# svip-lab/impersonator

Hardware: NVIDIA H100
Metric: frames/sec @256x256 (per-frame inference hot path) (higher is better)
Workload: dtype f16 main product + e4m3 correction products (hi/lo split), f32 accumulate

## Files before the change

impersonator_b200/csrc/conv_tc.cu:

```cuda
#include <cuda.h>

#include <stdlib.h>

#include <algorithm>
#include <new>

#include "common.cuh"

namespace {

constexpr int TILE_H = 16, TILE_W = 8;
constexpr int SWAP_N_TILE = 64;
constexpr int SWAP_TILE_H = 32;
constexpr int KCHUNK = 64;
constexpr int ROW_BYTES = TILE_W * 128;
constexpr int MAX_TAPS = 49;
constexpr int MAX_GROUP = 8;
constexpr int RING_BYTES = 200 * 1024;
constexpr int MAX_STAGES = 8;
constexpr int NUM_CONSUMERS = 256;
constexpr int NUM_THREADS = NUM_CONSUMERS + 32;
constexpr int MAX_N_TILE = 128;
static_assert(2 * 2 * (TILE_H + MAX_GROUP - 1) * ROW_BYTES + 2 * 2 * MAX_N_TILE * 128 <= RING_BYTES,
              "every plan needs two A and two B entries in the ring");
static_assert(2 * 2 * (SWAP_TILE_H + MAX_GROUP - 1) * ROW_BYTES + 2 * 2 * SWAP_N_TILE * 128 <= RING_BYTES,
              "every swapped plan needs two A and two B entries in the ring");
static_assert(SWAP_N_TILE * (SWAP_TILE_H * TILE_W) == MAX_N_TILE * (TILE_H * TILE_W), "same accumulator budget");

__host__ __device__ constexpr int tile_rows(int n_tile) { return n_tile == SWAP_N_TILE ? SWAP_TILE_H : TILE_H; }

struct ConvParams {
    CUtensorMap a_hi[4];
    CUtensorMap a_lo[4];
    CUtensorMap w_hi;
    CUtensorMap w_lo;
    int n_img, tiles_y, tiles_x, n_tiles_n;
    int dom_h, dom_w;
    int ntaps, chunks0, chunks1;
    signed char dy[MAX_TAPS], dx[MAX_TAPS], tmap[MAX_TAPS];
    short wtap[MAX_TAPS];
    int ngroups;
    signed char g_first[MAX_TAPS], g_cnt[MAX_TAPS];
    int a_rows;
    int a_stages, b_stages;
    float* out; int out_h, out_w, cout;
    int oy_mul, oy_add, ox_mul, ox_add;
    double* stats;
    float out_scale;
    int phase_cols;
};

template <int N_TILE, bool SPLIT>
struct Cfg {
    static constexpr int B_BYTES = N_TILE * 128;
    static constexpr int B_STAGE_BYTES = B_BYTES * (SPLIT ? 2 : 1);
    static constexpr int BAR_BYTES = 4 * MAX_STAGES * 8;
    static constexpr int STATS_BYTES = 8 * N_TILE * 8;
    static constexpr int SMEM_BYTES = 1024 + RING_BYTES + BAR_BYTES + STATS_BYTES;
    static_assert(B_STAGE_BYTES % 1024 == 0, "B entries must keep the 1024-byte swizzle alignment");
    static_assert(SMEM_BYTES <= 227 * 1024, "exceeds the shared memory of a block");
};

__device__ __forceinline__ uint32_t smem_u32(const void* p) { return (uint32_t)__cvta_generic_to_shared(p); }

__device__ __forceinline__ void mbar_init(uint64_t* bar, uint32_t count) {
    asm volatile("mbarrier.init.shared::cta.b64 [%0], %1;" ::"r"(smem_u32(bar)), "r"(count));
}
__device__ __forceinline__ void mbar_expect_tx(uint64_t* bar, uint32_t bytes) {
    asm volatile("mbarrier.arrive.expect_tx.shared::cta.b64 _, [%0], %1;" ::"r"(smem_u32(bar)), "r"(bytes) : "memory");
}
__device__ __forceinline__ void mbar_arrive(uint64_t* bar) {
    asm volatile("mbarrier.arrive.shared::cta.b64 _, [%0];" ::"r"(smem_u32(bar)) : "memory");
// ... 61 lines not shown
}
template <> __device__ __forceinline__ void wgmma_e4m3<16>(float* d, uint64_t da, uint64_t db) {
    asm volatile("{\n\t.reg .pred p;\n\tsetp.ne.b32 p, %10, 0;\n\t"
                 "wgmma.mma_async.sync.aligned.m64n16k32.f32.e4m3.e4m3 {%0, %1, %2, %3, %4, %5, %6, %7}, %8, %9, p, 1, 1;\n\t}"
                 : "+f"(d[0]), "+f"(d[1]), "+f"(d[2]), "+f"(d[3]), "+f"(d[4]), "+f"(d[5]), "+f"(d[6]), "+f"(d[7])
                 : "l"(da), "l"(db), "r"(1));
}
template <> __device__ __forceinline__ void wgmma_e4m3<32>(float* d, uint64_t da, uint64_t db) {
    asm volatile("{\n\t.reg .pred p;\n\tsetp.ne.b32 p, %18, 0;\n\t"
                 "wgmma.mma_async.sync.aligned.m64n32k32.f32.e4m3.e4m3 {%0, %1, %2, %3, %4, %5, %6, %7, %8, %9, %10, %11, %12, %13, %14, %15}, %16, %17, p, 1, 1;\n\t}"
                 : "+f"(d[0]), "+f"(d[1]), "+f"(d[2]), "+f"(d[3]), "+f"(d[4]), "+f"(d[5]), "+f"(d[6]), "+f"(d[7]), "+f"(d[8]), "+f"(d[9]), "+f"(d[10]), "+f"(d[11]), "+f"(d[12]), "+f"(d[13]), "+f"(d[14]), "+f"(d[15])
                 : "l"(da), "l"(db), "r"(1));
}
template <> __device__ __forceinline__ void wgmma_e4m3<128>(float* d, uint64_t da, uint64_t db) {
    asm volatile("{\n\t.reg .pred p;\n\tsetp.ne.b32 p, %66, 0;\n\t"
                 "wgmma.mma_async.sync.aligned.m64n128k32.f32.e4m3.e4m3 {%0, %1, %2, %3, %4, %5, %6, %7, %8, %9, %10, %11, %12, %13, %14, %15, %16, %17, %18, %19, %20, %21, %22, %23, %24, %25, %26, %27, %28, %29, %30, %31, %32, %33, %34, %35, %36, %37, %38, %39, %40, %41, %42, %43, %44, %45, %46, %47, %48, %49, %50, %51, %52, %53, %54, %55, %56, %57, %58, %59, %60, %61, %62, %63}, %64, %65, p, 1, 1;\n\t}"
                 : "+f"(d[0]), "+f"(d[1]), "+f"(d[2]), "+f"(d[3]), "+f"(d[4]), "+f"(d[5]), "+f"(d[6]), "+f"(d[7]), "+f"(d[8]), "+f"(d[9]), "+f"(d[10]), "+f"(d[11]), "+f"(d[12]), "+f"(d[13]), "+f"(d[14]), "+f"(d[15]), "+f"(d[16]), "+f"(d[17]), "+f"(d[18]), "+f"(d[19]), "+f"(d[20]), "+f"(d[21]), "+f"(d[22]), "+f"(d[23]), "+f"(d[24]), "+f"(d[25]), "+f"(d[26]), "+f"(d[27]), "+f"(d[28]), "+f"(d[29]), "+f"(d[30]), "+f"(d[31]), "+f"(d[32]), "+f"(d[33]), "+f"(d[34]), "+f"(d[35]), "+f"(d[36]), "+f"(d[37]), "+f"(d[38]), "+f"(d[39]), "+f"(d[40]), "+f"(d[41]), "+f"(d[42]), "+f"(d[43]), "+f"(d[44]), "+f"(d[45]), "+f"(d[46]), "+f"(d[47]), "+f"(d[48]), "+f"(d[49]), "+f"(d[50]), "+f"(d[51]), "+f"(d[52]), "+f"(d[53]), "+f"(d[54]), "+f"(d[55]), "+f"(d[56]), "+f"(d[57]), "+f"(d[58]), "+f"(d[59]), "+f"(d[60]), "+f"(d[61]), "+f"(d[62]), "+f"(d[63])
                 : "l"(da), "l"(db), "r"(1));
}

__device__ __forceinline__ void consumer_sync() { asm volatile("bar.sync 1, 256;" ::: "memory"); }

struct TileCoord {
    int n_idx, img, y0, x0;
};
template <int TH>
__device__ __forceinline__ TileCoord decode_tile(const ConvParams& P, int tile, int m_tiles) {
    TileCoord t;
    t.n_idx = tile / m_tiles;
    const int m_idx = tile % m_tiles;
    t.img = m_idx / (P.tiles_y * P.tiles_x);
    const int rem = m_idx % (P.tiles_y * P.tiles_x);
    t.y0 = (rem / P.tiles_x) * TH; t.x0 = (rem % P.tiles_x) * TILE_W;
    return t;
}

template <int N_TILE>
__device__ __forceinline__ void warp_tile_stats(const float* acc, bool v0, bool v1, int warp, unsigned lane, float2* s_stats)
{
#pragma unroll
    for (int j = 0; j < N_TILE / 8; j++) {
        const float a0 = v0 ? acc[4 * j] : 0.f, a1 = v0 ? acc[4 * j + 1] : 0.f;
        const float b0 = v1 ? acc[4 * j + 2] : 0.f, b1 = v1 ? acc[4 * j + 3] : 0.f;
        float s0 = a0 + b0, s1 = a1 + b1, q0 = a0 * a0 + b0 * b0, q1 = a1 * a1 + b1 * b1;
#pragma unroll
        for (int off = 4; off <= 16; off <<= 1) {
            s0 += __shfl_xor_sync(0xffffffffu, s0, off); s1 += __shfl_xor_sync(0xffffffffu, s1, off);
            q0 += __shfl_xor_sync(0xffffffffu, q0, off); q1 += __shfl_xor_sync(0xffffffffu, q1, off);
        }
        if (lane < 4) {
            s_stats[warp * N_TILE + 8 * j + 2 * lane] = make_float2(s0, q0);
            s_stats[warp * N_TILE + 8 * j + 2 * lane + 1] = make_float2(s1, q1);
        }
    }
}

template <int N_TILE, int PARTS = 8>
__device__ __forceinline__ void flush_tile_stats(const ConvParams& P, const float2* s_stats, int img, int n_idx)
{
    consumer_sync();
    for (int col = threadIdx.x; col < N_TILE; col += NUM_CONSUMERS) {
        float s = 0.f, q = 0.f;
#pragma unroll
        for (int w = 0; w < PARTS; w++) { const float2 v = s_stats[w * N_TILE + col]; s += v.x; q += v.y; }
        int ch = n_idx * N_TILE + col;
        if (P.phase_cols > 0) ch %= P.phase_cols;
        double* dst = P.stats + 2 * ((size_t)img * P.cout + ch);
        atomicAdd(dst, (double)s);
        atomicAdd(dst + 1, (double)q);
    }
    consumer_sync();
}

template <int N_TILE>
__device__ __forceinline__ void epilogue_plain(const ConvParams& P, float* acc, const TileCoord& t, int warp, unsigned lane,
                                               float2* s_stats)
{
    const int tx = (int)(lane >> 2), x = t.x0 + tx;
    const int y[2] = {t.y0 + 2 * warp, t.y0 + 2 * warp + 1};
    const bool valid[2] = {y[0] < P.dom_h && x < P.dom_w, y[1] < P.dom_h && x < P.dom_w};
    if (P.out_scale != 1.f) {
#pragma unroll
        for (int i = 0; i < N_TILE / 2; i++) acc[i] *= P.out_scale;
    }
    if (P.out) {
        const int out_w_c = P.out_w * P.cout;
#pragma unroll
        for (int h = 0; h < 2; h++) {
            if (!valid[h]) continue;
            float* optr = P.out + (((size_t)t.img * P.out_h + (P.oy_mul * y[h] + P.oy_add)) * P.out_w + (P.ox_mul * x + P.ox_add)) * P.cout
                        + (size_t)t.n_idx * N_TILE;
#pragma unroll
            for (int j = 0; j < N_TILE / 8; j++) {
                const int c = 8 * j + 2 * (int)(lane & 3);
                float* o = optr + c;
                if (P.phase_cols > 0) {
                    const int col = t.n_idx * N_TILE + c, ph = col / P.phase_cols;
                    o = P.out + (((size_t)t.img * P.out_h + 2 * y[h]) * P.out_w + 2 * x) * P.cout
                      + (size_t)(ph >> 1) * out_w_c + (ph & 1) * P.cout + (col - ph * P.phase_cols);
                }
                *reinterpret_cast<float2*>(o) = make_float2(acc[4 * j + 2 * h], acc[4 * j + 2 * h + 1]);
            }
        }
    }
    if (P.stats) {
        warp_tile_stats<N_TILE>(acc, valid[0], valid[1], warp, lane, s_stats);
        flush_tile_stats<N_TILE>(P, s_stats, t.img, t.n_idx);
    }
}

__device__ __forceinline__ void epilogue_swapped(const ConvParams& P, float* acc, const TileCoord& t, int warp, unsigned lane,
                                                 float2* s_stats)
{
    constexpr int N = SWAP_N_TILE;
    const int wg = warp >> 2;
    const int c0 = 16 * (warp & 3) + (int)(lane >> 2);
    const int y0 = t.y0 + 16 * wg, x0 = t.x0 + 2 * (int)(lane & 3);
    const int rows = P.dom_h - y0;
    const bool vx[2] = {x0 < P.dom_w, x0 + 1 < P.dom_w};
    if (P.out_scale != 1.f) {
#pragma unroll
        for (int i = 0; i < 64; i++) acc[i] *= P.out_scale;
    }
    if (P.out) {
        float* obase = P.out + (size_t)t.n_idx * N + c0;
#pragma unroll
        for (int j = 0; j < 16; j++) {
            if (j >= rows) break;
            const size_t orow = ((size_t)t.img * P.out_h + (P.oy_mul * (y0 + j) + P.oy_add)) * P.out_w;
#pragma unroll
            for (int e = 0; e < 2; e++) {
                if (!vx[e]) continue;
                float* o = obase + (orow + (P.ox_mul * (x0 + e) + P.ox_add)) * P.cout;
                o[0] = acc[4 * j + e];
                o[8] = acc[4 * j + 2 + e];
            }
        }
    }
    if (P.stats) {
        float s[2] = {0.f, 0.f}, q[2] = {0.f, 0.f};
#pragma unroll
        for (int j = 0; j < 16; j++) {
#pragma unroll
            for (int e = 0; e < 2; e++) {
                const bool v = j < rows && vx[e];
#pragma unroll
                for (int h = 0; h < 2; h++) {
                    const float a = v ? acc[4 * j + 2 * h + e] : 0.f;
                    s[h] += a; q[h] += a * a;
                }
            }
        }
#pragma unroll
        for (int h = 0; h < 2; h++) {
#pragma unroll
            for (int off = 1; off <= 2; off <<= 1) {
// ... 36 lines not shown
    const int a_stage_bytes = a_op_bytes * (SPLIT ? 2 : 1);
    uint8_t* b_ring = smem + P.a_stages * a_stage_bytes;
    uint64_t* a_full = reinterpret_cast<uint64_t*>(smem + RING_BYTES);
    uint64_t* a_empty = a_full + MAX_STAGES;
    uint64_t* b_full = a_empty + MAX_STAGES;
    uint64_t* b_empty = b_full + MAX_STAGES;
    float2* s_stats = reinterpret_cast<float2*>(smem + RING_BYTES + C::BAR_BYTES);

    const int warp = threadIdx.x >> 5;
    const unsigned lane = threadIdx.x & 31;

    if (threadIdx.x == 0) {
        for (int s = 0; s < P.a_stages; s++) { mbar_init(a_full + s, 1); mbar_init(a_empty + s, NUM_CONSUMERS / 32); }
        for (int s = 0; s < P.b_stages; s++) { mbar_init(b_full + s, 1); mbar_init(b_empty + s, NUM_CONSUMERS / 32); }
        fence_barrier_init();
        fence_proxy_async();
    }
    __syncthreads();
    lwb::pdl_wait();
    lwb::pdl_trigger();

    const int nchunks = P.chunks0 + P.chunks1;
    const int m_tiles = P.n_img * P.tiles_y * P.tiles_x;
    const int total = m_tiles * P.n_tiles_n;

    if (warp == NUM_CONSUMERS / 32) {
        if (elect_one()) {
            asm volatile("prefetch.tensormap [%0];" :: "l"(&P.a_hi[0]) : "memory");
            asm volatile("prefetch.tensormap [%0];" :: "l"(&P.w_hi) : "memory");
            if (SPLIT) {
                asm volatile("prefetch.tensormap [%0];" :: "l"(&P.a_lo[0]) : "memory");
                asm volatile("prefetch.tensormap [%0];" :: "l"(&P.w_lo) : "memory");
            }
        }
        int as = 0, bs = 0; uint32_t aph = 0, bph = 0;
        for (int tile = blockIdx.x; tile < total; tile += gridDim.x) {
            const TileCoord t = decode_tile<TH>(P, tile, m_tiles);
            for (int g = 0; g < P.ngroups; g++) {
                const int first = P.g_first[g], cnt = P.g_cnt[g];
                const int xx = t.x0 + P.dx[first], yy = t.y0 + P.dy[first];
                for (int chunk = 0; chunk < nchunks; chunk++) {
                    const bool second = chunk >= P.chunks0;
                    const int mi = second ? 1 : P.tmap[first];
                    const int c0 = (second ? chunk - P.chunks0 : chunk) * KCHUNK;
                    mbar_wait(a_empty + as, aph ^ 1);
                    uint8_t* sa = smem + as * a_stage_bytes;
                    if (elect_one()) {
                        mbar_expect_tx(a_full + as, (uint32_t)a_stage_bytes);
                        tma_load_4d(&P.a_hi[mi], sa, a_full + as, c0, xx, yy, t.img);
                        if (SPLIT) tma_load_4d(&P.a_lo[mi], sa + a_op_bytes, a_full + as, c0, xx, yy, t.img);
                    }
                    __syncwarp();
                    if (++as == P.a_stages) { as = 0; aph ^= 1; }
                    for (int i = 0; i < cnt; i++) {
                        mbar_wait(b_empty + bs, bph ^ 1);
                        uint8_t* sb = b_ring + bs * C::B_STAGE_BYTES;
                        const int wt = P.wtap[first + i];
                        if (elect_one()) {
                            mbar_expect_tx(b_full + bs, (uint32_t)C::B_STAGE_BYTES);
                            tma_load_3d(&P.w_hi, sb, b_full + bs, chunk * KCHUNK, t.n_idx * N_TILE, wt);
                            if (SPLIT) tma_load_3d(&P.w_lo, sb + C::B_BYTES, b_full + bs, chunk * KCHUNK, t.n_idx * N_TILE, wt);
                        }
                        __syncwarp();
                        if (++bs == P.b_stages) { bs = 0; bph ^= 1; }
                    }
                }
            }
        }
    } else if (warp < NUM_CONSUMERS / 32) {
        const uint32_t smem_base = smem_u32(smem);
        const uint32_t b_base = smem_u32(b_ring);
        const uint32_t a_row0 = (uint32_t)(warp >> 2) * (TH / 2) * ROW_BYTES;
        float acc[ACC];
        float acc8[MODE == MODE_F8 ? ACC : 1];
        int as = 0, bs = 0; uint32_t aph = 0, bph = 0;
        for (int tile = blockIdx.x; tile < total; tile += gridDim.x) {
            const TileCoord t = decode_tile<TH>(P, tile, m_tiles);
#pragma unroll
            for (int i = 0; i < ACC; i++) acc[i] = 0.f;
#pragma unroll
            for (int i = 0; i < (MODE == MODE_F8 ? ACC : 1); i++) acc8[i] = 0.f;
            int prev_b = -1, prev_a = -1;
            for (int g = 0; g < P.ngroups; g++) {
                const int cnt = P.g_cnt[g];
                for (int chunk = 0; chunk < nchunks; chunk++) {
                    mbar_wait(a_full + as, aph);
                    const uint32_t a_hi = smem_base + as * a_stage_bytes + a_row0;
                    for (int i = 0; i < cnt; i++) {
                        mbar_wait(b_full + bs, bph);
                        const uint32_t ai = a_hi + i * ROW_BYTES, al = ai + a_op_bytes;
                        const uint32_t b_hi = b_base + bs * C::B_STAGE_BYTES, b_lo = b_hi + C::B_BYTES;
                        wgmma_fence();
#pragma unroll
                        for (int k = 0; k < KCHUNK / 16; k++) {
                            const uint64_t da = make_desc(ai + k * 32), db = make_desc(b_hi + k * 32);
                            mma_f16<N_TILE, SWAP>(acc, da, db);
                            if constexpr (MODE == MODE_F8) {
                                mma_e4m3<N_TILE, SWAP>(acc8, make_desc(al + k * 32), make_desc(b_lo + k * 32));
                            } else if constexpr (MODE == MODE_FP16X3) {
                                mma_f16<N_TILE, SWAP>(acc, da, make_desc(b_lo + k * 32));
                                mma_f16<N_TILE, SWAP>(acc, make_desc(al + k * 32), db);
                            }
                        }
                        wgmma_commit();
                        if (prev_b >= 0) {
                            wgmma_wait<1>();
// ... 96 lines not shown
    switch (L.n_tile) {
        case 16:  return launch_one<16>(L, st);
        case 32:  return launch_one<32>(L, st);
        case 64:  return launch_one<64>(L, st);
        case 128: return launch_one<128>(L, st);
    }
    lwb::set_error("conv_tc: unsupported N tile %d", L.n_tile);
    return LWB_E_UNSUPPORTED;
}

int pick_n_tile(int cout, int forced)
{
    if (forced > 0) return forced > MAX_N_TILE && forced % MAX_N_TILE == 0 ? MAX_N_TILE : forced;
    if (cout % 128 == 0) return 128;
    if (cout % 64 == 0) return 64;
    if (cout % 32 == 0) return 32;
    if (cout % 16 == 0) return 16;
    return -1;
}

}

struct lwb_conv_plan {
    int num;
    Launch launches[4];
};

static int map_nhwc(CUtensorMap* m, const uint16_t* base, int n, int h, int w, int c, int rows)
{
    const uint64_t dims[4] = {(uint64_t)c, (uint64_t)w, (uint64_t)h, (uint64_t)n};
    const uint64_t str[3] = {(uint64_t)c * 2, (uint64_t)w * c * 2, (uint64_t)h * w * c * 2};
    const uint32_t box[4] = {(uint32_t)KCHUNK, TILE_W, (uint32_t)rows, 1};
    return encode_map(m, base, 4, dims, str, box);
}
static int map_nhwc_parity(CUtensorMap* m, const uint16_t* base, int n, int h, int w, int c, int py, int px, int rows)
{
    const uint64_t dims[4] = {(uint64_t)c, (uint64_t)((w - px + 1) / 2), (uint64_t)((h - py + 1) / 2), (uint64_t)n};
    const uint64_t str[3] = {(uint64_t)2 * c * 2, (uint64_t)2 * w * c * 2, (uint64_t)h * w * c * 2};
    const uint32_t box[4] = {(uint32_t)KCHUNK, TILE_W, (uint32_t)rows, 1};
    return encode_map(m, base + ((size_t)py * w + px) * c, 4, dims, str, box);
}

static void group_taps(ConvParams& p, int tile_h)
{
    int order[MAX_TAPS];
    for (int t = 0; t < p.ntaps; t++) order[t] = t;
    std::stable_sort(order, order + p.ntaps, [&](int a, int b) {
        if (p.tmap[a] != p.tmap[b]) return p.tmap[a] < p.tmap[b];
        if (p.dx[a] != p.dx[b]) return p.dx[a] < p.dx[b];
        return p.dy[a] < p.dy[b];
    });
    const ConvParams src = p;
    int longest = 0;
    p.ngroups = 0;
    for (int t = 0; t < p.ntaps; t++) {
        const int o = order[t];
        p.dy[t] = src.dy[o]; p.dx[t] = src.dx[o]; p.tmap[t] = src.tmap[o]; p.wtap[t] = src.wtap[o];
        const bool joins = t > 0 && p.tmap[t] == p.tmap[t - 1] && p.dx[t] == p.dx[t - 1] && p.dy[t] == p.dy[t - 1] + 1 &&
                           p.g_cnt[p.ngroups - 1] < MAX_GROUP;
        if (!joins) { p.g_first[p.ngroups] = (signed char)t; p.g_cnt[p.ngroups] = 0; p.ngroups++; }
        p.g_cnt[p.ngroups - 1]++;
        longest = std::max(longest, (int)p.g_cnt[p.ngroups - 1]);
    }
    p.a_rows = tile_h + longest - 1;
}

static void pick_rings(ConvParams& p, int n_tile, bool split)
{
    const int ops = split ? 2 : 1;
    const int a_bytes = p.a_rows * ROW_BYTES * ops, b_bytes = n_tile * 128 * ops;
    const int longest = p.a_rows - tile_rows(n_tile) + 1;
    int best = 0;
    for (int a = 2; a <= MAX_STAGES; a++) {
        const int b = std::min(MAX_STAGES, (RING_BYTES - a * a_bytes) / b_bytes);
        if (b < 2) break;
        if (std::min(a * longest, b) > best) { best = std::min(a * longest, b); p.a_stages = a; p.b_stages = b; }
    }
}

extern "C" int lwb_conv_plan_create(const lwb_conv_desc* d,
                                    const uint16_t* x0_hi, const uint16_t* x0_lo,
                                    const uint16_t* x1_hi, const uint16_t* x1_lo,
                                    const uint16_t* w_hi, const uint16_t* w_lo,
                                    float* out_raw, double* stats, lwb_conv_plan** plan_out)
{
    LWB_CHECK_ARG(d && x0_hi && w_hi && out_raw && plan_out, "null pointer");
    const bool split = d->split != 0;
    const bool f8 = d->split == 2;
    LWB_CHECK_ARG(d->split >= 0 && d->split <= 2, "split must be 0, 1 or 2");
    LWB_CHECK_ARG(!split || (x0_lo && w_lo), "split mode needs the lo operands");
    LWB_CHECK_ARG(!f8 || (!d->rowk && !d->halo), "the fp8 lo mode is not available for row-K / halo plans");
    LWB_CHECK_ARG(d->n > 0 && d->h_in > 0 && d->w_in > 0 && d->cout > 0, "non-positive size");
    LWB_CHECK_ARG(d->cout % 16 == 0, "cout must be a multiple of 16");
    LWB_CHECK_ARG(!f8 || (d->w_exp >= -40 && d->w_exp <= 60), "w_exp out of range");
    int n_tile = pick_n_tile(d->cout, d->n_tile);
    LWB_CHECK_ARG(n_tile > 0 && d->cout % n_tile == 0, "no N tile divides cout");
    if (d->halo) {
        LWB_CHECK_ARG(d->stride == 1 && !d->transposed && d->dil == 1, "halo mode needs stride 1, dilation 1, not transposed");
        if (d->rowk) LWB_CHECK_ARG(d->kw <= 8 && d->cin0 == 8 && d->cin1 == 0 && d->row_pitch >= d->w_in + 8, "row-K shape");
        else         LWB_CHECK_ARG(d->kw <= 9 && (d->kw & 1) && (d->kh & 1), "halo mode needs an odd kernel, kw <= 9, with 'same' padding (kh/2, kw/2)");
    }

    const int sms = lwb::sm_count();
    lwb_conv_plan* plan = new (std::nothrow) lwb_conv_plan();
    LWB_CHECK_ARG(plan, "out of host memory");
    plan->num = 0;
    int rc = LWB_OK;
    auto fail = [&](int code) { delete plan; return code; };

    auto finish = [&](Launch& L, int dom_h, int dom_w) {
        ConvParams& p = L.p;
        p.n_img = d->n;
        p.dom_h = dom_h; p.dom_w = dom_w;
        p.tiles_y = lwb::ceil_div(dom_h, tile_rows(n_tile)); p.tiles_x = lwb::ceil_div(dom_w, TILE_W);
        p.n_tiles_n = d->cout / n_tile;
        p.out = out_raw; p.out_h = d->h_out; p.out_w = d->w_out; p.cout = d->cout;
        p.stats = stats;
        p.out_scale = f8 ? ldexpf(1.f, -d->w_exp) : 1.f;
        L.n_tile = n_tile; L.mode = d->split;
        pick_rings(p, n_tile, split);
        const long total = (long)p.n_img * p.tiles_y * p.tiles_x * p.n_tiles_n;
        L.grid = (int)(total < sms ? total : sms);
    };

    if (d->rowk) {
        LWB_CHECK_ARG(d->stride == 1 && !d->transposed && d->kw <= 8 && d->cin0 == 8 && d->cin1 == 0, "row-K needs stride 1, kw <= 8, 8 channels");
        LWB_CHECK_ARG(d->h_out == d->h_in && d->w_out == d->w_in && d->row_pitch >= d->w_in + 8, "row-K shape");
        Launch& L = plan->launches[plan->num++];
        memset(&L.p, 0, sizeof(L.p));
        L.p.ntaps = d->kh; L.p.chunks0 = 1; L.p.chunks1 = 0;
        for (int ky = 0; ky < d->kh; ky++) { L.p.dy[ky] = (signed char)ky; L.p.dx[ky] = 0; L.p.tmap[ky] = 0; L.p.wtap[ky] = (short)ky; }
        group_taps(L.p, tile_rows(n_tile));
        const int hp = d->h_in + d->kh - 1;
        const uint64_t dims[4] = {64, (uint64_t)d->w_in, (uint64_t)hp, (uint64_t)d->n};
        const uint64_t str[3] = {16, (uint64_t)d->row_pitch * 16, (uint64_t)hp * d->row_pitch * 16};
        const uint32_t box[4] = {KCHUNK, TILE_W, (uint32_t)L.p.a_rows, 1};
        if ((rc = encode_map(&L.p.a_hi[0], x0_hi, 4, dims, str, box)) != LWB_OK) return fail(rc);
        if (split && (rc = encode_map(&L.p.a_lo[0], x0_lo, 4, dims, str, box)) != LWB_OK) return fail(rc);
        const uint64_t wd[3] = {64, (uint64_t)d->cout, (uint64_t)d->kh};
        const uint64_t ws[2] = {128, (uint64_t)d->cout * 128};
        const uint32_t wb[3] = {KCHUNK, (uint32_t)n_tile, 1};
        if ((rc = encode_map(&L.p.w_hi, w_hi, 3, wd, ws, wb)) != LWB_OK) return fail(rc);
        if (split && (rc = encode_map(&L.p.w_lo, w_lo, 3, wd, ws, wb)) != LWB_OK) return fail(rc);
        L.p.oy_mul = 1; L.p.ox_mul = 1; L.p.oy_add = 0; L.p.ox_add = 0;
        finish(L, d->h_out, d->w_out);
        *plan_out = plan;
        return LWB_OK;
    }

    LWB_CHECK_ARG(d->cin0 % KCHUNK == 0 && d->cin1 % KCHUNK == 0 && d->cin0 > 0, "input channels must be multiples of 64");
    LWB_CHECK_ARG(d->cin1 == 0 || (x1_hi && (!split || x1_lo)), "second input missing");
    const int cin_total = d->cin0 + d->cin1;
    const int ntaps_w = d->kh * d->kw;
    LWB_CHECK_ARG(ntaps_w <= MAX_TAPS, "too many filter taps");
    const uint64_t wd[3] = {(uint64_t)cin_total, (uint64_t)d->cout, (uint64_t)ntaps_w};
    const uint64_t ws[2] = {(uint64_t)cin_total * 2, (uint64_t)d->cout * cin_total * 2};
    const uint32_t wb[3] = {(uint32_t)KCHUNK, (uint32_t)n_tile, 1};

    if (d->transposed == 2) {
        LWB_CHECK_ARG(d->kh == 3 && d->kw == 3 && d->stride == 2 && d->pad == 1 && d->cin1 == 0, "transposed conv: only k3 s2 p1 op1");
        LWB_CHECK_ARG(d->h_out == 2 * d->h_in && d->w_out == 2 * d->w_in, "transposed conv output must be 2x input");
        const int ncols = 4 * d->cout;
        n_tile = MAX_N_TILE;
        LWB_CHECK_ARG(d->cout % 32 == 0 && ncols % n_tile == 0, "merged transposed conv needs cout in multiples of 32");
        Launch& L = plan->launches[plan->num++];
        memset(&L.p, 0, sizeof(L.p));
        for (int t = 0; t < 4; t++) { L.p.dy[t] = (signed char)(t >> 1); L.p.dx[t] = (signed char)(t & 1); L.p.tmap[t] = 0; L.p.wtap[t] = (short)t; }
        L.p.ntaps = 4; L.p.chunks0 = d->cin0 / KCHUNK; L.p.chunks1 = 0;
        group_taps(L.p, tile_rows(n_tile));
        if ((rc = map_nhwc(&L.p.a_hi[0], x0_hi, d->n, d->h_in, d->w_in, d->cin0, L.p.a_rows)) != LWB_OK) return fail(rc);
        if (split && (rc = map_nhwc(&L.p.a_lo[0], x0_lo, d->n, d->h_in, d->w_in, d->cin0, L.p.a_rows)) != LWB_OK) return fail(rc);
        const uint64_t mwd[3] = {(uint64_t)cin_total, (uint64_t)ncols, 4};
        const uint64_t mws[2] = {(uint64_t)cin_total * 2, (uint64_t)ncols * cin_total * 2};
        const uint32_t mwb[3] = {(uint32_t)KCHUNK, (uint32_t)n_tile, 1};
        if ((rc = encode_map(&L.p.w_hi, w_hi, 3, mwd, mws, mwb)) != LWB_OK) return fail(rc);
        if (split && (rc = encode_map(&L.p.w_lo, w_lo, 3, mwd, mws, mwb)) != LWB_OK) return fail(rc);
        L.p.oy_mul = 2; L.p.ox_mul = 2; L.p.oy_add = 0; L.p.ox_add = 0;
        finish(L, d->h_in, d->w_in);
        L.p.phase_cols = d->cout;
        L.p.n_tiles_n = ncols / n_tile;
        const long total = (long)L.p.n_img * L.p.tiles_y * L.p.tiles_x * L.p.n_tiles_n;
        L.grid = (int)(total < sms ? total : sms);
        *plan_out = plan;
        return LWB_OK;
    }

    if (d->transposed) {
        LWB_CHECK_ARG(d->kh == 3 && d->kw == 3 && d->stride == 2 && d->pad == 1 && d->cin1 == 0, "transposed conv: only k3 s2 p1 op1");
        LWB_CHECK_ARG(d->h_out == 2 * d->h_in && d->w_out == 2 * d->w_in, "transposed conv output must be 2x input");
        for (int a = 0; a < 2; a++) for (int b = 0; b < 2; b++) {
            Launch& L = plan->launches[plan->num++];
            memset(&L.p, 0, sizeof(L.p));
            const int ky_list[2][2] = {{1, -1}, {2, 0}}, d_list[2][2] = {{0, 0}, {0, 1}}, cnt[2] = {1, 2};
            int t = 0;
            for (int i = 0; i < cnt[a]; i++) for (int j = 0; j < cnt[b]; j++) {
                L.p.dy[t] = (signed char)d_list[a][i]; L.p.dx[t] = (signed char)d_list[b][j];
                L.p.tmap[t] = 0; L.p.wtap[t] = (short)(ky_list[a][i] * 3 + ky_list[b][j]);
                t++;
            }
            L.p.ntaps = t; L.p.chunks0 = d->cin0 / KCHUNK; L.p.chunks1 = 0;
            group_taps(L.p, tile_rows(n_tile));
            if ((rc = map_nhwc(&L.p.a_hi[0], x0_hi, d->n, d->h_in, d->w_in, d->cin0, L.p.a_rows)) != LWB_OK) return fail(rc);
            if (split && (rc = map_nhwc(&L.p.a_lo[0], x0_lo, d->n, d->h_in, d->w_in, d->cin0, L.p.a_rows)) != LWB_OK) return fail(rc);
            if ((rc = encode_map(&L.p.w_hi, w_hi, 3, wd, ws, wb)) != LWB_OK) return fail(rc);
            if (split && (rc = encode_map(&L.p.w_lo, w_lo, 3, wd, ws, wb)) != LWB_OK) return fail(rc);
            L.p.oy_mul = 2; L.p.ox_mul = 2; L.p.oy_add = a; L.p.ox_add = b;
            finish(L, d->h_in, d->w_in);
        }
        *plan_out = plan;
        return LWB_OK;
    }

    LWB_CHECK_ARG(d->stride == 1 || d->stride == 2, "stride must be 1 or 2");
    LWB_CHECK_ARG(d->stride == 1 || d->cin1 == 0, "concat input only with stride 1");
    Launch& L = plan->launches[plan->num++];
    memset(&L.p, 0, sizeof(L.p));
    int t = 0;
    for (int ky = 0; ky < d->kh; ky++) for (int kx = 0; kx < d->kw; kx++) {
        const int oy = ky * d->dil - d->pad, ox = kx * d->dil - (d->pad_w >= 0 ? d->pad_w : d->pad);
        if (oy < -127 || oy > 127 || ox < -127 || ox > 127) { lwb::set_error("conv_tc: tap offset out of range"); return fail(LWB_E_UNSUPPORTED); }
        if (d->stride == 1) {
            L.p.dy[t] = (signed char)oy; L.p.dx[t] = (signed char)ox; L.p.tmap[t] = 0;
        } else {
            const int py = ((oy % 2) + 2) % 2, px = ((ox % 2) + 2) % 2;
            L.p.dy[t] = (signed char)((oy - py) / 2); L.p.dx[t] = (signed char)((ox - px) / 2);
            L.p.tmap[t] = (signed char)(py * 2 + px);
        }
        L.p.wtap[t] = (short)t;
        t++;
    }
    L.p.ntaps = t; L.p.chunks0 = d->cin0 / KCHUNK; L.p.chunks1 = d->cin1 / KCHUNK;
    L.p.oy_mul = 1; L.p.ox_mul = 1; L.p.oy_add = 0; L.p.ox_add = 0;
    group_taps(L.p, tile_rows(n_tile));
    const int rows = L.p.a_rows;
    if (d->stride == 1) {
        if ((rc = map_nhwc(&L.p.a_hi[0], x0_hi, d->n, d->h_in, d->w_in, d->cin0, rows)) != LWB_OK) return fail(rc);
        if (split && (rc = map_nhwc(&L.p.a_lo[0], x0_lo, d->n, d->h_in, d->w_in, d->cin0, rows)) != LWB_OK) return fail(rc);
        if (d->cin1) {
            if ((rc = map_nhwc(&L.p.a_hi[1], x1_hi, d->n, d->h_in, d->w_in, d->cin1, rows)) != LWB_OK) return fail(rc);
            if (split && (rc = map_nhwc(&L.p.a_lo[1], x1_lo, d->n, d->h_in, d->w_in, d->cin1, rows)) != LWB_OK) return fail(rc);
        }
    } else {
        for (int py = 0; py < 2; py++) for (int px = 0; px < 2; px++) {
            if ((rc = map_nhwc_parity(&L.p.a_hi[py * 2 + px], x0_hi, d->n, d->h_in, d->w_in, d->cin0, py, px, rows)) != LWB_OK) return fail(rc);
            if (split && (rc = map_nhwc_parity(&L.p.a_lo[py * 2 + px], x0_lo, d->n, d->h_in, d->w_in, d->cin0, py, px, rows)) != LWB_OK) return fail(rc);
        }
    }
    if ((rc = encode_map(&L.p.w_hi, w_hi, 3, wd, ws, wb)) != LWB_OK) return fail(rc);
    if (split && (rc = encode_map(&L.p.w_lo, w_lo, 3, wd, ws, wb)) != LWB_OK) return fail(rc);
    finish(L, d->h_out, d->w_out);
    *plan_out = plan;
    return LWB_OK;
}

extern "C" int lwb_conv_plan_run(const lwb_conv_plan* plan, lwb_stream_t stream)
{
    LWB_CHECK_ARG(plan, "null plan");
    for (int i = 0; i < plan->num; i++) {
        const int rc = launch(plan->launches[i], (cudaStream_t)stream);
        if (rc != LWB_OK) return rc;
    }
    return LWB_OK;
}

extern "C" void lwb_conv_plan_destroy(lwb_conv_plan* plan) { delete plan; }

extern "C" int lwb_conv_plan_num_launches(const lwb_conv_plan* plan) { return plan ? plan->num : 0; }

extern "C" int lwb_conv2d_nhwc(const lwb_conv_desc* d,
                               const uint16_t* x0_hi, const uint16_t* x0_lo,
                               const uint16_t* x1_hi, const uint16_t* x1_lo,
                               const uint16_t* w_hi, const uint16_t* w_lo,
                               float* out_raw, double* stats, lwb_stream_t stream)
{
    lwb_conv_plan* plan = nullptr;
    int rc = lwb_conv_plan_create(d, x0_hi, x0_lo, x1_hi, x1_lo, w_hi, w_lo, out_raw, stats, &plan);
    if (rc != LWB_OK) return rc;
    rc = lwb_conv_plan_run(plan, stream);
    lwb_conv_plan_destroy(plan);
    return rc;
}
```

impersonator_b200/generator.py:

```python
import os

import torch
import torch.nn as nn

from . import graph as _graph
from . import kernels as K
from ._lib import LwbError


DEFAULT_PRECISION = "fp16f8"


_WEIGHTS_EPOCH = [0]
_PASS = [0]


def _new_pass():
    _PASS[0] += 1



def weights_epoch():
    return _WEIGHTS_EPOCH[0]


def precision_mode():
    return os.environ.get("LWB_PRECISION", DEFAULT_PRECISION)


def _sub_batches(B, enc_w, res_w, bg):
    try:
        n = min(2, int(os.environ.get("LWB_STREAMS", "2")))
    except ValueError:
        n = 1
    if n <= 1 or B % n or B // n < 4:
        return 1
    shared = all(t is None or t.shape[0] == 1 for t in list(enc_w) + list(res_w)) and (bg is None or bg.shape[0] == 1)
    return n if shared else 1


def _tc_heads():
    return os.environ.get("LWB_TC_HEADS", "1") != "0"


def _convt_merge():
    return os.environ.get("LWB_CONVT_MERGE", "1") != "0"


def merge_transposed_weight(wt):
    cin, cout = wt.shape[0], wt.shape[1]
    k_of = ({0: 1}, {0: 2, 1: 0})
    out = torch.zeros((4 * cout, cin, 2, 2), dtype=torch.float32, device=wt.device)
    for a in range(2):
        for b in range(2):
            ph = 2 * a + b
            for dy, ky in k_of[a].items():
                for dx, kx in k_of[b].items():
                    out[ph * cout:(ph + 1) * cout, :, dy, dx] = wt[:, :, ky, kx].t().float()
    return out


def fold_head_weights(w_img, w_att):
    w4 = torch.cat([w_img, w_att], dim=0).float()
    folded = w4.permute(3, 0, 1, 2).reshape(28, w4.shape[1], 7, 1)
    return torch.cat([folded, torch.zeros(4, w4.shape[1], 7, 1, dtype=folded.dtype, device=folded.device)], dim=0).contiguous()


def _split_mode(mod=None):
    mode = (getattr(mod, '_lwb_precision', None) if mod is not None else None) or precision_mode()
# ... 132 lines not shown
        self._raw = {}
        self.ws = None

    def _raw_buf(self, h, w, c):
        key = (h, w, c)
        if key not in self._raw:
            self._raw[key] = torch.empty((self.B, h, w, c), dtype=torch.float32, device=self.dev)
        return self._raw[key]

    def _make_layer(self, conv, norm, x0, x1=None, stride=1, transposed=False, rowk=False, row_pitch=0, h=None, w=None,
                    halo=False, weight=None, pad=None, n_tile=0, pad_w=None):
        L = _Layer()
        wt = (weight if weight is not None else conv.weight).detach()
        L.wsrc = None
        if rowk:
            L.w = K.pack_conv_weight_rowk(wt, split=min(self.split, 1))
            cout, kh, kw = wt.shape[0], wt.shape[2], wt.shape[3]
            d = K.make_conv_desc(self.B, h, w, 8, cout, kh, kw, stride=1, pad=kh // 2, split=min(self.split, 1),
                                 rowk=True, row_pitch=row_pitch, halo=halo)
        else:
            L.w = None
            cout = wt.shape[1] if transposed else wt.shape[0]
            kh, kw = wt.shape[2], wt.shape[3]
            merged = bool(transposed and _convt_merge() and cout <= 128 and cout % 32 == 0 and (kh, kw) == (3, 3))
            L.wsrc = (merge_transposed_weight(wt), False) if merged else (wt, transposed)
            cin0 = x0[0].shape[3]
            cin1 = x1[0].shape[3] if x1 is not None else 0
            d = K.make_conv_desc(self.B, h, w, cin0, cout, kh, kw, stride=stride,
                                 pad=(pad if pad is not None else conv.padding[0]),
                                 cin1=cin1, transposed=transposed, split=self.split, halo=halo, n_tile=n_tile, pad_w=pad_w)
            if merged:
                d.transposed = 2
        L.raw = self._raw_buf(d.h_out, d.w_out, cout)
        L.stats = (len(self._stats_slots), cout)
        self._stats_slots.append(cout)
        L.gamma = norm.weight.detach().float().contiguous() if norm is not None else None
        L.beta = norm.bias.detach().float().contiguous() if norm is not None else None
        L.plan = (d, x0, x1)
        self._layers.append(L)
        return L

    def _finalize(self):
        cmax = max(max(self._stats_slots), 16)
        nstat = len(self._stats_slots) * self.B * cmax * 2
        self._zero = torch.zeros(nstat * 8 + 4, dtype=torch.uint8, device=self.dev)
        self.stats = self._zero[:nstat * 8].view(torch.float64).view(len(self._stats_slots), self.B, cmax, 2)
        self.range_flag = self._zero[nstat * 8:].view(torch.int32)
        self.ws = torch.empty((self.B, cmax, 2), dtype=torch.float32, device=self.dev)
        pend = [L for L in self._layers if L.wsrc is not None]
        if pend:
            amax = [None] * len(pend)
            if self.split == 2:
                amax = torch.stack([L.wsrc[0].abs().max().float() for L in pend]).tolist()
            for L, a in zip(pend, amax):
                L.w = K.pack_conv_weight(L.wsrc[0], transposed=L.wsrc[1], split=self.split, absmax=a)
# ... 512 lines not shown
```

Baseline: 2033.

## Run transposed conv as one phase-aware persistent launch with per-phase taps

Replaces the four separate sub-pixel phase launches (and the merged 2x2 variant with zero-padded taps) with a single launch. The tile index now encodes the phase, and each phase runs only its own tap groups and writes to its own output offset. The aim is to cut launch overhead and tail imbalance across the phases while skipping the zero taps of the merged form. Phases now have unequal tap counts (1, 2, 2, 4) inside one persistent schedule, which can leave per-tile work unbalanced. The Python side stops building merged weights, so the non-stacked path with original 3x3 weights is used.

```diff
diff --git a/impersonator_b200/csrc/conv_tc.cu b/impersonator_b200/csrc/conv_tc.cu
--- a/impersonator_b200/csrc/conv_tc.cu
+++ b/impersonator_b200/csrc/conv_tc.cu
@@ -43,11 +43,13 @@
     signed char g_first[MAX_TAPS], g_cnt[MAX_TAPS];
     int a_rows;
     int a_stages, b_stages;
+    int nphases;
+    signed char ph_g0[5], ph_oy[4], ph_ox[4];
+    int ph_wn[4];
     float* out; int out_h, out_w, cout;
-    int oy_mul, oy_add, ox_mul, ox_add;
+    int oy_mul, ox_mul;
     double* stats;
     float out_scale;
-    int phase_cols;
 };
 
 template <int N_TILE, bool SPLIT>
@@ -155,13 +157,18 @@
 __device__ __forceinline__ void consumer_sync() { asm volatile("bar.sync 1, 256;" ::: "memory"); }
 
 struct TileCoord {
-    int n_idx, img, y0, x0;
+    int ph, n_idx, img, y0, x0;
+    int oy_add, ox_add;
 };
 template <int TH>
 __device__ __forceinline__ TileCoord decode_tile(const ConvParams& P, int tile, int m_tiles) {
     TileCoord t;
-    t.n_idx = tile / m_tiles;
-    const int m_idx = tile % m_tiles;
+    const int per_phase = m_tiles * P.n_tiles_n;
+    t.ph = tile / per_phase;
+    const int r = tile - t.ph * per_phase;
+    t.oy_add = P.ph_oy[t.ph]; t.ox_add = P.ph_ox[t.ph];
+    t.n_idx = r / m_tiles;
+    const int m_idx = r - t.n_idx * m_tiles;
     t.img = m_idx / (P.tiles_y * P.tiles_x);
     const int rem = m_idx % (P.tiles_y * P.tiles_x);
     t.y0 = (rem / P.tiles_x) * TH; t.x0 = (rem % P.tiles_x) * TILE_W;
@@ -196,9 +203,7 @@
         float s = 0.f, q = 0.f;
 #pragma unroll
         for (int w = 0; w < PARTS; w++) { const float2 v = s_stats[w * N_TILE + col]; s += v.x; q += v.y; }
-        int ch = n_idx * N_TILE + col;
-        if (P.phase_cols > 0) ch %= P.phase_cols;
-        double* dst = P.stats + 2 * ((size_t)img * P.cout + ch);
+        double* dst = P.stats + 2 * ((size_t)img * P.cout + n_idx * N_TILE + col);
         atomicAdd(dst, (double)s);
         atomicAdd(dst + 1, (double)q);
     }
@@ -217,22 +222,15 @@
         for (int i = 0; i < N_TILE / 2; i++) acc[i] *= P.out_scale;
     }
     if (P.out) {
-        const int out_w_c = P.out_w * P.cout;
 #pragma unroll
         for (int h = 0; h < 2; h++) {
             if (!valid[h]) continue;
-            float* optr = P.out + (((size_t)t.img * P.out_h + (P.oy_mul * y[h] + P.oy_add)) * P.out_w + (P.ox_mul * x + P.ox_add)) * P.cout
+            float* optr = P.out + (((size_t)t.img * P.out_h + (P.oy_mul * y[h] + t.oy_add)) * P.out_w + (P.ox_mul * x + t.ox_add)) * P.cout
                         + (size_t)t.n_idx * N_TILE;
 #pragma unroll
             for (int j = 0; j < N_TILE / 8; j++) {
                 const int c = 8 * j + 2 * (int)(lane & 3);
-                float* o = optr + c;
-                if (P.phase_cols > 0) {
-                    const int col = t.n_idx * N_TILE + c, ph = col / P.phase_cols;
-                    o = P.out + (((size_t)t.img * P.out_h + 2 * y[h]) * P.out_w + 2 * x) * P.cout
-                      + (size_t)(ph >> 1) * out_w_c + (ph & 1) * P.cout + (col - ph * P.phase_cols);
-                }
-                *reinterpret_cast<float2*>(o) = make_float2(acc[4 * j + 2 * h], acc[4 * j + 2 * h + 1]);
+                *reinterpret_cast<float2*>(optr + c) = make_float2(acc[4 * j + 2 * h], acc[4 * j + 2 * h + 1]);
             }
         }
     }
@@ -260,11 +258,11 @@
 #pragma unroll
         for (int j = 0; j < 16; j++) {
             if (j >= rows) break;
-            const size_t orow = ((size_t)t.img * P.out_h + (P.oy_mul * (y0 + j) + P.oy_add)) * P.out_w;
+            const size_t orow = ((size_t)t.img * P.out_h + (P.oy_mul * (y0 + j) + t.oy_add)) * P.out_w;
 #pragma unroll
             for (int e = 0; e < 2; e++) {
                 if (!vx[e]) continue;
-                float* o = obase + (orow + (P.ox_mul * (x0 + e) + P.ox_add)) * P.cout;
+                float* o = obase + (orow + (P.ox_mul * (x0 + e) + t.ox_add)) * P.cout;
                 o[0] = acc[4 * j + e];
                 o[8] = acc[4 * j + 2 + e];
             }
@@ -347,7 +345,7 @@
 
     const int nchunks = P.chunks0 + P.chunks1;
     const int m_tiles = P.n_img * P.tiles_y * P.tiles_x;
-    const int total = m_tiles * P.n_tiles_n;
+    const int total = m_tiles * P.n_tiles_n * P.nphases;
 
     if (warp == NUM_CONSUMERS / 32) {
         if (elect_one()) {
@@ -361,7 +359,8 @@
         int as = 0, bs = 0; uint32_t aph = 0, bph = 0;
         for (int tile = blockIdx.x; tile < total; tile += gridDim.x) {
             const TileCoord t = decode_tile<TH>(P, tile, m_tiles);
-            for (int g = 0; g < P.ngroups; g++) {
+            const int wn = P.ph_wn[t.ph] + t.n_idx * N_TILE;
+            for (int g = P.ph_g0[t.ph]; g < P.ph_g0[t.ph + 1]; g++) {
                 const int first = P.g_first[g], cnt = P.g_cnt[g];
                 const int xx = t.x0 + P.dx[first], yy = t.y0 + P.dy[first];
                 for (int chunk = 0; chunk < nchunks; chunk++) {
@@ -383,8 +382,8 @@
                         const int wt = P.wtap[first + i];
                         if (elect_one()) {
                             mbar_expect_tx(b_full + bs, (uint32_t)C::B_STAGE_BYTES);
-                            tma_load_3d(&P.w_hi, sb, b_full + bs, chunk * KCHUNK, t.n_idx * N_TILE, wt);
-                            if (SPLIT) tma_load_3d(&P.w_lo, sb + C::B_BYTES, b_full + bs, chunk * KCHUNK, t.n_idx * N_TILE, wt);
+                            tma_load_3d(&P.w_hi, sb, b_full + bs, chunk * KCHUNK, wn, wt);
+                            if (SPLIT) tma_load_3d(&P.w_lo, sb + C::B_BYTES, b_full + bs, chunk * KCHUNK, wn, wt);
                         }
                         __syncwarp();
                         if (++bs == P.b_stages) { bs = 0; bph ^= 1; }
@@ -406,7 +405,7 @@
 #pragma unroll
             for (int i = 0; i < (MODE == MODE_F8 ? ACC : 1); i++) acc8[i] = 0.f;
             int prev_b = -1, prev_a = -1;
-            for (int g = 0; g < P.ngroups; g++) {
+            for (int g = P.ph_g0[t.ph]; g < P.ph_g0[t.ph + 1]; g++) {
                 const int cnt = P.g_cnt[g];
                 for (int chunk = 0; chunk < nchunks; chunk++) {
                     mbar_wait(a_full + as, aph);
@@ -549,8 +548,7 @@
 }
 
 struct lwb_conv_plan {
-    int num;
-    Launch launches[4];
+    Launch launch;
 };
 
 static int map_nhwc(CUtensorMap* m, const uint16_t* base, int n, int h, int w, int c, int rows)
@@ -568,28 +566,41 @@
     return encode_map(m, base + ((size_t)py * w + px) * c, 4, dims, str, box);
 }
 
-static void group_taps(ConvParams& p, int tile_h)
+static void group_taps(ConvParams& p, int tile_h, int nphases, const int* phase_first)
 {
     int order[MAX_TAPS];
     for (int t = 0; t < p.ntaps; t++) order[t] = t;
-    std::stable_sort(order, order + p.ntaps, [&](int a, int b) {
-        if (p.tmap[a] != p.tmap[b]) return p.tmap[a] < p.tmap[b];
-        if (p.dx[a] != p.dx[b]) return p.dx[a] < p.dx[b];
-        return p.dy[a] < p.dy[b];
-    });
+    for (int ph = 0; ph < nphases; ph++) {
+        std::stable_sort(order + phase_first[ph], order + phase_first[ph + 1], [&](int a, int b) {
+            if (p.tmap[a] != p.tmap[b]) return p.tmap[a] < p.tmap[b];
+            if (p.dx[a] != p.dx[b]) return p.dx[a] < p.dx[b];
+            return p.dy[a] < p.dy[b];
+        });
+    }
     const ConvParams src = p;
     int longest = 0;
     p.ngroups = 0;
-    for (int t = 0; t < p.ntaps; t++) {
-        const int o = order[t];
-        p.dy[t] = src.dy[o]; p.dx[t] = src.dx[o]; p.tmap[t] = src.tmap[o]; p.wtap[t] = src.wtap[o];
-        const bool joins = t > 0 && p.tmap[t] == p.tmap[t - 1] && p.dx[t] == p.dx[t - 1] && p.dy[t] == p.dy[t - 1] + 1 &&
-                           p.g_cnt[p.ngroups - 1] < MAX_GROUP;
-        if (!joins) { p.g_first[p.ngroups] = (signed char)t; p.g_cnt[p.ngroups] = 0; p.ngroups++; }
-        p.g_cnt[p.ngroups - 1]++;
-        longest = std::max(longest, (int)p.g_cnt[p.ngroups - 1]);
-    }
+    p.nphases = nphases;
+    for (int ph = 0; ph < nphases; ph++) {
+        p.ph_g0[ph] = (signed char)p.ngroups;
+        for (int t = phase_first[ph]; t < phase_first[ph + 1]; t++) {
+            const int o = order[t];
+            p.dy[t] = src.dy[o]; p.dx[t] = src.dx[o]; p.tmap[t] = src.tmap[o]; p.wtap[t] = src.wtap[o];
+            const bool joins = t > phase_first[ph] && p.tmap[t] == p.tmap[t - 1] && p.dx[t] == p.dx[t - 1] &&
+                               p.dy[t] == p.dy[t - 1] + 1 && p.g_cnt[p.ngroups - 1] < MAX_GROUP;
+            if (!joins) { p.g_first[p.ngroups] = (signed char)t; p.g_cnt[p.ngroups] = 0; p.ngroups++; }
+            p.g_cnt[p.ngroups - 1]++;
+            longest = std::max(longest, (int)p.g_cnt[p.ngroups - 1]);
+        }
+    }
+    p.ph_g0[nphases] = (signed char)p.ngroups;
     p.a_rows = tile_h + longest - 1;
+}
+
+static void group_taps(ConvParams& p, int tile_h)
+{
+    const int phase_first[2] = {0, p.ntaps};
+    group_taps(p, tile_h, 1, phase_first);
 }
 
 static void pick_rings(ConvParams& p, int n_tile, bool split)
@@ -612,6 +623,7 @@
                                     float* out_raw, double* stats, lwb_conv_plan** plan_out)
 {
     LWB_CHECK_ARG(d && x0_hi && w_hi && out_raw && plan_out, "null pointer");
+    LWB_CHECK_ARG(d->transposed >= 0 && d->transposed <= 2, "transposed must be 0, 1 or 2");
     const bool split = d->split != 0;
     const bool f8 = d->split == 2;
     LWB_CHECK_ARG(d->split >= 0 && d->split <= 2, "split must be 0, 1 or 2");
@@ -631,11 +643,12 @@
     const int sms = lwb::sm_count();
     lwb_conv_plan* plan = new (std::nothrow) lwb_conv_plan();
     LWB_CHECK_ARG(plan, "out of host memory");
-    plan->num = 0;
+    Launch& L = plan->launch;
+    memset(&L.p, 0, sizeof(L.p));
     int rc = LWB_OK;
     auto fail = [&](int code) { delete plan; return code; };
 
-    auto finish = [&](Launch& L, int dom_h, int dom_w) {
+    auto finish = [&](int dom_h, int dom_w) {
         ConvParams& p = L.p;
         p.n_img = d->n;
         p.dom_h = dom_h; p.dom_w = dom_w;
@@ -646,15 +659,13 @@
         p.out_scale = f8 ? ldexpf(1.f, -d->w_exp) : 1.f;
         L.n_tile = n_tile; L.mode = d->split;
         pick_rings(p, n_tile, split);
-        const long total = (long)p.n_img * p.tiles_y * p.tiles_x * p.n_tiles_n;
+        const long total = (long)p.n_img * p.tiles_y * p.tiles_x * p.n_tiles_n * p.nphases;
         L.grid = (int)(total < sms ? total : sms);
     };
 
     if (d->rowk) {
         LWB_CHECK_ARG(d->stride == 1 && !d->transposed && d->kw <= 8 && d->cin0 == 8 && d->cin1 == 0, "row-K needs stride 1, kw <= 8, 8 channels");
         LWB_CHECK_ARG(d->h_out == d->h_in && d->w_out == d->w_in && d->row_pitch >= d->w_in + 8, "row-K shape");
-        Launch& L = plan->launches[plan->num++];
-        memset(&L.p, 0, sizeof(L.p));
         L.p.ntaps = d->kh; L.p.chunks0 = 1; L.p.chunks1 = 0;
         for (int ky = 0; ky < d->kh; ky++) { L.p.dy[ky] = (signed char)ky; L.p.dx[ky] = 0; L.p.tmap[ky] = 0; L.p.wtap[ky] = (short)ky; }
         group_taps(L.p, tile_rows(n_tile));
@@ -669,8 +680,8 @@
         const uint32_t wb[3] = {KCHUNK, (uint32_t)n_tile, 1};
         if ((rc = encode_map(&L.p.w_hi, w_hi, 3, wd, ws, wb)) != LWB_OK) return fail(rc);
         if (split && (rc = encode_map(&L.p.w_lo, w_lo, 3, wd, ws, wb)) != LWB_OK) return fail(rc);
-        L.p.oy_mul = 1; L.p.ox_mul = 1; L.p.oy_add = 0; L.p.ox_add = 0;
-        finish(L, d->h_out, d->w_out);
+        L.p.oy_mul = 1; L.p.ox_mul = 1;
+        finish(d->h_out, d->w_out);
         *plan_out = plan;
         return LWB_OK;
     }
@@ -684,64 +695,42 @@
     const uint64_t ws[2] = {(uint64_t)cin_total * 2, (uint64_t)d->cout * cin_total * 2};
     const uint32_t wb[3] = {(uint32_t)KCHUNK, (uint32_t)n_tile, 1};
 
-    if (d->transposed == 2) {
-        LWB_CHECK_ARG(d->kh == 3 && d->kw == 3 && d->stride == 2 && d->pad == 1 && d->cin1 == 0, "transposed conv: only k3 s2 p1 op1");
-        LWB_CHECK_ARG(d->h_out == 2 * d->h_in && d->w_out == 2 * d->w_in, "transposed conv output must be 2x input");
-        const int ncols = 4 * d->cout;
-        n_tile = MAX_N_TILE;
-        LWB_CHECK_ARG(d->cout % 32 == 0 && ncols % n_tile == 0, "merged transposed conv needs cout in multiples of 32");
-        Launch& L = plan->launches[plan->num++];
-        memset(&L.p, 0, sizeof(L.p));
-        for (int t = 0; t < 4; t++) { L.p.dy[t] = (signed char)(t >> 1); L.p.dx[t] = (signed char)(t & 1); L.p.tmap[t] = 0; L.p.wtap[t] = (short)t; }
-        L.p.ntaps = 4; L.p.chunks0 = d->cin0 / KCHUNK; L.p.chunks1 = 0;
-        group_taps(L.p, tile_rows(n_tile));
-        if ((rc = map_nhwc(&L.p.a_hi[0], x0_hi, d->n, d->h_in, d->w_in, d->cin0, L.p.a_rows)) != LWB_OK) return fail(rc);
-        if (split && (rc = map_nhwc(&L.p.a_lo[0], x0_lo, d->n, d->h_in, d->w_in, d->cin0, L.p.a_rows)) != LWB_OK) return fail(rc);
-        const uint64_t mwd[3] = {(uint64_t)cin_total, (uint64_t)ncols, 4};
-        const uint64_t mws[2] = {(uint64_t)cin_total * 2, (uint64_t)ncols * cin_total * 2};
-        const uint32_t mwb[3] = {(uint32_t)KCHUNK, (uint32_t)n_tile, 1};
-        if ((rc = encode_map(&L.p.w_hi, w_hi, 3, mwd, mws, mwb)) != LWB_OK) return fail(rc);
-        if (split && (rc = encode_map(&L.p.w_lo, w_lo, 3, mwd, mws, mwb)) != LWB_OK) return fail(rc);
-        L.p.oy_mul = 2; L.p.ox_mul = 2; L.p.oy_add = 0; L.p.ox_add = 0;
-        finish(L, d->h_in, d->w_in);
-        L.p.phase_cols = d->cout;
-        L.p.n_tiles_n = ncols / n_tile;
-        const long total = (long)L.p.n_img * L.p.tiles_y * L.p.tiles_x * L.p.n_tiles_n;
-        L.grid = (int)(total < sms ? total : sms);
-        *plan_out = plan;
-        return LWB_OK;
-    }
-
     if (d->transposed) {
         LWB_CHECK_ARG(d->kh == 3 && d->kw == 3 && d->stride == 2 && d->pad == 1 && d->cin1 == 0, "transposed conv: only k3 s2 p1 op1");
         LWB_CHECK_ARG(d->h_out == 2 * d->h_in && d->w_out == 2 * d->w_in, "transposed conv output must be 2x input");
-        for (int a = 0; a < 2; a++) for (int b = 0; b < 2; b++) {
-            Launch& L = plan->launches[plan->num++];
-            memset(&L.p, 0, sizeof(L.p));
-            const int ky_list[2][2] = {{1, -1}, {2, 0}}, d_list[2][2] = {{0, 0}, {0, 1}}, cnt[2] = {1, 2};
-            int t = 0;
+        const bool stacked = d->transposed == 2;
+        const int phases[4][2] = {{1, 1}, {0, 1}, {1, 0}, {0, 0}};
+        const int ky_list[2][2] = {{1, -1}, {2, 0}}, d_list[2][2] = {{0, 0}, {0, 1}}, cnt[2] = {1, 2};
+        int phase_first[5], t = 0;
+        for (int ph = 0; ph < 4; ph++) {
+            const int a = phases[ph][0], b = phases[ph][1];
+            phase_first[ph] = t;
+            L.p.ph_oy[ph] = (signed char)a; L.p.ph_ox[ph] = (signed char)b;
+            L.p.ph_wn[ph] = stacked ? (2 * a + b) * d->cout : 0;
             for (int i = 0; i < cnt[a]; i++) for (int j = 0; j < cnt[b]; j++) {
                 L.p.dy[t] = (signed char)d_list[a][i]; L.p.dx[t] = (signed char)d_list[b][j];
-                L.p.tmap[t] = 0; L.p.wtap[t] = (short)(ky_list[a][i] * 3 + ky_list[b][j]);
+                L.p.tmap[t] = 0;
+                L.p.wtap[t] = (short)(stacked ? d_list[a][i] * 2 + d_list[b][j] : ky_list[a][i] * 3 + ky_list[b][j]);
                 t++;
             }
-            L.p.ntaps = t; L.p.chunks0 = d->cin0 / KCHUNK; L.p.chunks1 = 0;
-            group_taps(L.p, tile_rows(n_tile));
-            if ((rc = map_nhwc(&L.p.a_hi[0], x0_hi, d->n, d->h_in, d->w_in, d->cin0, L.p.a_rows)) != LWB_OK) return fail(rc);
-            if (split && (rc = map_nhwc(&L.p.a_lo[0], x0_lo, d->n, d->h_in, d->w_in, d->cin0, L.p.a_rows)) != LWB_OK) return fail(rc);
-            if ((rc = encode_map(&L.p.w_hi, w_hi, 3, wd, ws, wb)) != LWB_OK) return fail(rc);
-            if (split && (rc = encode_map(&L.p.w_lo, w_lo, 3, wd, ws, wb)) != LWB_OK) return fail(rc);
-            L.p.oy_mul = 2; L.p.ox_mul = 2; L.p.oy_add = a; L.p.ox_add = b;
-            finish(L, d->h_in, d->w_in);
-        }
+        }
+        phase_first[4] = t;
+        L.p.ntaps = t; L.p.chunks0 = d->cin0 / KCHUNK; L.p.chunks1 = 0;
+        group_taps(L.p, tile_rows(n_tile), 4, phase_first);
+        if ((rc = map_nhwc(&L.p.a_hi[0], x0_hi, d->n, d->h_in, d->w_in, d->cin0, L.p.a_rows)) != LWB_OK) return fail(rc);
+        if (split && (rc = map_nhwc(&L.p.a_lo[0], x0_lo, d->n, d->h_in, d->w_in, d->cin0, L.p.a_rows)) != LWB_OK) return fail(rc);
+        const uint64_t swd[3] = {(uint64_t)cin_total, (uint64_t)4 * d->cout, 4};
+        const uint64_t sws[2] = {(uint64_t)cin_total * 2, (uint64_t)4 * d->cout * cin_total * 2};
+        if ((rc = encode_map(&L.p.w_hi, w_hi, 3, stacked ? swd : wd, stacked ? sws : ws, wb)) != LWB_OK) return fail(rc);
+        if (split && (rc = encode_map(&L.p.w_lo, w_lo, 3, stacked ? swd : wd, stacked ? sws : ws, wb)) != LWB_OK) return fail(rc);
+        L.p.oy_mul = 2; L.p.ox_mul = 2;
+        finish(d->h_in, d->w_in);
         *plan_out = plan;
         return LWB_OK;
     }
 
     LWB_CHECK_ARG(d->stride == 1 || d->stride == 2, "stride must be 1 or 2");
     LWB_CHECK_ARG(d->stride == 1 || d->cin1 == 0, "concat input only with stride 1");
-    Launch& L = plan->launches[plan->num++];
-    memset(&L.p, 0, sizeof(L.p));
     int t = 0;
     for (int ky = 0; ky < d->kh; ky++) for (int kx = 0; kx < d->kw; kx++) {
         const int oy = ky * d->dil - d->pad, ox = kx * d->dil - (d->pad_w >= 0 ? d->pad_w : d->pad);
@@ -757,7 +746,7 @@
         t++;
     }
     L.p.ntaps = t; L.p.chunks0 = d->cin0 / KCHUNK; L.p.chunks1 = d->cin1 / KCHUNK;
-    L.p.oy_mul = 1; L.p.ox_mul = 1; L.p.oy_add = 0; L.p.ox_add = 0;
+    L.p.oy_mul = 1; L.p.ox_mul = 1;
     group_taps(L.p, tile_rows(n_tile));
     const int rows = L.p.a_rows;
     if (d->stride == 1) {
@@ -775,7 +764,7 @@
     }
     if ((rc = encode_map(&L.p.w_hi, w_hi, 3, wd, ws, wb)) != LWB_OK) return fail(rc);
     if (split && (rc = encode_map(&L.p.w_lo, w_lo, 3, wd, ws, wb)) != LWB_OK) return fail(rc);
-    finish(L, d->h_out, d->w_out);
+    finish(d->h_out, d->w_out);
     *plan_out = plan;
     return LWB_OK;
 }
@@ -783,16 +772,12 @@
 extern "C" int lwb_conv_plan_run(const lwb_conv_plan* plan, lwb_stream_t stream)
 {
     LWB_CHECK_ARG(plan, "null plan");
-    for (int i = 0; i < plan->num; i++) {
-        const int rc = launch(plan->launches[i], (cudaStream_t)stream);
-        if (rc != LWB_OK) return rc;
-    }
-    return LWB_OK;
+    return launch(plan->launch, (cudaStream_t)stream);
 }
 
 extern "C" void lwb_conv_plan_destroy(lwb_conv_plan* plan) { delete plan; }
 
-extern "C" int lwb_conv_plan_num_launches(const lwb_conv_plan* plan) { return plan ? plan->num : 0; }
+extern "C" int lwb_conv_plan_num_launches(const lwb_conv_plan* plan) { return plan ? 1 : 0; }
 
 extern "C" int lwb_conv2d_nhwc(const lwb_conv_desc* d,
                                const uint16_t* x0_hi, const uint16_t* x0_lo,
diff --git a/impersonator_b200/generator.py b/impersonator_b200/generator.py
--- a/impersonator_b200/generator.py
+++ b/impersonator_b200/generator.py
@@ -41,10 +41,6 @@
 
 def _tc_heads():
     return os.environ.get("LWB_TC_HEADS", "1") != "0"
-
-
-def _convt_merge():
-    return os.environ.get("LWB_CONVT_MERGE", "1") != "0"
 
 
 def merge_transposed_weight(wt):
@@ -223,15 +219,12 @@
             L.w = None
             cout = wt.shape[1] if transposed else wt.shape[0]
             kh, kw = wt.shape[2], wt.shape[3]
-            merged = bool(transposed and _convt_merge() and cout <= 128 and cout % 32 == 0 and (kh, kw) == (3, 3))
-            L.wsrc = (merge_transposed_weight(wt), False) if merged else (wt, transposed)
+            L.wsrc = (wt, transposed)
             cin0 = x0[0].shape[3]
             cin1 = x1[0].shape[3] if x1 is not None else 0
             d = K.make_conv_desc(self.B, h, w, cin0, cout, kh, kw, stride=stride,
                                  pad=(pad if pad is not None else conv.padding[0]),
                                  cin1=cin1, transposed=transposed, split=self.split, halo=halo, n_tile=n_tile, pad_w=pad_w)
-            if merged:
-                d.transposed = 2
         L.raw = self._raw_buf(d.h_out, d.w_out, cout)
         L.stats = (len(self._stats_slots), cout)
         self._stats_slots.append(cout)
```

Measured after the change: 2095, median of 6. 3.1% higher.
